# kotaro-kinoshita/yomitoku

Hardware: AMD Instinct MI355X
Metric: pages/sec (DocumentAnalyzer @1600x1200, lite model set) (higher is better)
Workload: dtype f32 held as two scaled fp16 planes per operand on the MFMA pipe: 3 x v_mfma_f32_32x32x16_f16 per product tile (products to 2^-21, below the fp32 accumulation's own rounding), fp32 accumulate, fp32 activations in HBM; attention, LayerNorm, the fused greedy step and every grid-starved launch exact fp3

## Files before the change

yomitoku_amd/csrc/ymk_api.cpp:

```cpp
#include "../../include/ymk.h"
#include "ymk_common.h"
#include "ymk_det.h"
#include "ymk_seq.h"

namespace ymk {
const std::string& last_error();
void dbnet_forward(Model* m, const float* x, int n, int h, int w, float* prob, hipStream_t s);
void parseq_forward(Model* m, const float* x, int B, int W, float* logits, int* out_len, int* ar_steps, hipStream_t s);
void parseq_forward_groups(Model* m, const float* const* x, const int* b, const int* w, int ng, float* logits, int* out_len,
                           int* ar_steps, hipStream_t s);
void parseq_dims(Model* m, int* num_steps, int* num_classes);
Model* create_parseq();
Model* create_rtdetr();
void rtdetr_forward(Model* m, const float* x, int B, int H, int W, float* logits, float* boxes, hipStream_t s);
void row_maxprob(hipStream_t s, const float* logits, int rows, int C, int* ids, float* probs);
void prof_begin();
void prof_end(double* ms, double* flop, int64_t* launches);
double prof_bytes();
int64_t prof_launch_table(double* ms, double* flop, double* bytes, double* products, int64_t capacity);
bool gemm_takes_astat(int M, int K, const ConvW& w, bool with_res, int ld);
bool conv_debug_option(const std::string& key, int value);
bool parseq_debug_option(const std::string& key, int value);
bool decstep_debug_option(const std::string& key, int value);
bool conv_split_debug_option(const std::string& key, int value);
bool conv_split_stat(const std::string& key, long long* value);
void amax_check_counters(long long* out4);
}

struct ymk_model {
  ymk::Model* impl = nullptr;
  int device = 0;
};

#include <dlfcn.h>
namespace {
struct Roctx {
  int (*push)(const char*) = nullptr;
  int (*pop)() = nullptr;
  Roctx() {
    const char* on = std::getenv("YMK_ROCTX");
    if (on == nullptr || on[0] == '\0' || on[0] == '0') return;
    for (const char* name : {"librocprofiler-sdk-roctx.so", "libroctx64.so"}) {
      if (void* h = dlopen(name, RTLD_NOW | RTLD_GLOBAL)) {
        push = reinterpret_cast<int (*)(const char*)>(dlsym(h, "roctxRangePushA"));
        pop = reinterpret_cast<int (*)()>(dlsym(h, "roctxRangePop"));
        if (push && pop) return;
        push = nullptr;
        pop = nullptr;
      }
    }
  }
};
struct RoctxRange {
  explicit RoctxRange(const char* name) {
    static Roctx r;
    pop_ = r.pop;
    if (r.push) (void)r.push(name);
    else pop_ = nullptr;
  }
  ~RoctxRange() {
    if (pop_) (void)pop_();
  }
  int (*pop_)() = nullptr;
};
}

#define YMK_API_BEGIN try {
#define YMK_API_END                                 \
  return 0;                                         \
  }                                                 \
  catch (const std::exception& e) {                 \
    ymk::set_error(e.what());                       \
    return 1;                                       \
  }                                                 \
  catch (...) {                                     \
    ymk::set_error("unknown C++ exception");        \
    return 2;                                       \
  }

extern "C" {

int ymk_version(void) { return 100; }

const char* ymk_last_error(void) { return ymk::last_error().c_str(); }

int ymk_device_count(void) {
  int n = 0;
  if (hipGetDeviceCount(&n) != hipSuccess) return -1;
  return n;
}

ymk_model* ymk_model_create(const char* kind, int device) {
  try {
    YMK_CHECK(kind != nullptr, "kind is null");
    YMK_HIP(hipSetDevice(device));
    std::string k(kind);
    ymk::Model* impl = nullptr;
    if (k == "dbnet") impl = ymk::create_dbnet();
    else if (k == "parseq") impl = ymk::create_parseq();
    else if (k == "rtdetr") impl = ymk::create_rtdetr();
    else throw ymk::Error("unknown model kind: " + k);
    auto* m = new ymk_model();
    m->impl = impl;
    m->device = device;
    return m;
  } catch (const std::exception& e) {
// ... 32 lines not shown
int ymk_model_finalize(ymk_model* m) {
  YMK_API_BEGIN
  RoctxRange roctx_range("ymk_model_finalize");
  YMK_CHECK(m, "null model");
  YMK_HIP(hipSetDevice(m->device));
  m->impl->finalize();
  m->impl->prebuild_split();
  if (!ymk::debug_hazard_no_finalize_sync()) YMK_HIP(hipDeviceSynchronize());
  YMK_API_END
}

int ymk_model_reserve(ymk_model* m, int n, int h, int w, void* stream) {
  YMK_API_BEGIN
  RoctxRange roctx_range("ymk_model_reserve");
  YMK_CHECK(m && m->impl, "null argument");
  YMK_HIP(hipSetDevice(m->device));
  m->impl->reserve(n, h, w, (hipStream_t)stream);
  YMK_API_END
}

int64_t ymk_model_weight_bytes(const ymk_model* m) { return m ? (int64_t)m->impl->pool.bytes() : -1; }
int64_t ymk_model_workspace_bytes(const ymk_model* m) { return m ? (int64_t)m->impl->arena.capacity() : -1; }

int ymk_dbnet_forward(ymk_model* m, const float* x_dev, int n, int h, int w, float* prob_dev, void* stream) {
  YMK_API_BEGIN
  RoctxRange roctx_range("ymk_dbnet_forward");
  YMK_CHECK(m && x_dev && prob_dev, "null argument");
  YMK_HIP(hipSetDevice(m->device));
  ymk::dbnet_forward(m->impl, x_dev, n, h, w, prob_dev, (hipStream_t)stream);
  YMK_API_END
}

int ymk_parseq_dims(ymk_model* m, int* num_steps, int* num_classes) {
  YMK_API_BEGIN
  YMK_CHECK(m && num_steps && num_classes, "null argument");
  ymk::parseq_dims(m->impl, num_steps, num_classes);
  YMK_API_END
}

int ymk_parseq_forward(ymk_model* m, const float* x_dev, int b, int w, float* logits_dev, int* out_len, int* ar_steps,
                       void* stream) {
  YMK_API_BEGIN
  RoctxRange roctx_range("ymk_parseq_forward");
  YMK_CHECK(m && x_dev && logits_dev && out_len && ar_steps, "null argument");
  YMK_HIP(hipSetDevice(m->device));
  ymk::parseq_forward(m->impl, x_dev, b, w, logits_dev, out_len, ar_steps, (hipStream_t)stream);
  YMK_API_END
}

int ymk_parseq_forward_groups(ymk_model* m, const float* const* x_dev, const int* b, const int* w, int n_groups,
                              float* logits_dev, int* out_len, int* ar_steps, void* stream) {
  YMK_API_BEGIN
  RoctxRange roctx_range("ymk_parseq_forward_groups");
  YMK_CHECK(m && x_dev && b && w && logits_dev && out_len && ar_steps, "null argument");
  YMK_HIP(hipSetDevice(m->device));
  ymk::parseq_forward_groups(m->impl, x_dev, b, w, n_groups, logits_dev, out_len, ar_steps, (hipStream_t)stream);
  YMK_API_END
}

int ymk_parseq_token_stats(const float* logits_dev, int rows, int num_classes, int* ids_dev, float* probs_dev,
                           void* stream) {
  YMK_API_BEGIN
  RoctxRange roctx_range("ymk_parseq_token_stats");
  YMK_CHECK(logits_dev && ids_dev && probs_dev, "null argument");
  ymk::row_maxprob((hipStream_t)stream, logits_dev, rows, num_classes, ids_dev, probs_dev);
  YMK_API_END
}

int ymk_rtdetr_forward(ymk_model* m, const float* x_dev, int b, int h, int w, float* logits_dev, float* boxes_dev,
                       void* stream) {
  YMK_API_BEGIN
  RoctxRange roctx_range("ymk_rtdetr_forward");
  YMK_CHECK(m && x_dev && logits_dev && boxes_dev, "null argument");
  YMK_HIP(hipSetDevice(m->device));
  ymk::rtdetr_forward(m->impl, x_dev, b, h, w, logits_dev, boxes_dev, (hipStream_t)stream);
  YMK_API_END
}

int ymk_debug_option(const char* key, int value) {
  YMK_API_BEGIN
  YMK_CHECK(key != nullptr, "null key");
  const std::string k(key);
  YMK_CHECK(ymk::conv_debug_option(k, value) || ymk::parseq_debug_option(k, value) || ymk::decstep_debug_option(k, value) ||
                ymk::conv_split_debug_option(k, value),
            "unknown debug option: " + k);
  YMK_API_END
}

int ymk_stat(const char* key, int64_t* value) {
  YMK_API_BEGIN
  YMK_CHECK(key != nullptr && value != nullptr, "null argument");
  long long v = 0;
  YMK_CHECK(ymk::conv_split_stat(std::string(key), &v) || ymk::runtime_stat(std::string(key), &v), std::string("unknown counter: ") + key);
  *value = v;
  YMK_API_END
}

int ymk_amax_check_counters(int64_t* out4) {
  YMK_API_BEGIN
  YMK_CHECK(out4 != nullptr, "null argument");
  long long v[4];
  ymk::amax_check_counters(v);
  for (int i = 0; i < 4; ++i) out4[i] = v[i];
  YMK_API_END
}

int ymk_prof_begin(void) {
  YMK_API_BEGIN
  ymk::prof_begin();
  YMK_API_END
}

int ymk_prof_end(double* conv_ms, double* conv_flop, int64_t* conv_launches) {
  YMK_API_BEGIN
  YMK_CHECK(conv_ms && conv_flop && conv_launches, "null argument");
  ymk::prof_end(conv_ms, conv_flop, conv_launches);
  YMK_API_END
}

int ymk_prof_bytes(double* conv_bytes) {
  YMK_API_BEGIN
  YMK_CHECK(conv_bytes, "null argument");
  *conv_bytes = ymk::prof_bytes();
  YMK_API_END
}

int ymk_prof_launch_table(double* ms, double* flop, double* bytes, double* mfma_products, int64_t capacity, int64_t* count) {
  YMK_API_BEGIN
  YMK_CHECK(count != nullptr && capacity >= 0 && (capacity == 0 || (ms && flop && bytes && mfma_products)), "null argument");
  *count = ymk::prof_launch_table(ms, flop, bytes, mfma_products, capacity);
  YMK_API_END
}

int ymk_op_conv2d(const float* x_dev, int n, int h, int w, int c, const float* w_host_oihw, int cout, int cin, int kh,
                  int kw, const float* scale_host, const float* bias_host, const float* res_dev, int stride, int pad,
                  int dil, int act, int tap4, float* y_dev, void* stream) {
  YMK_API_BEGIN
  using namespace ymk;
  DevicePool pool;
  ConvW cw;
  cw.cout = cout;
  cw.cin = tap4 ? 4 : cin;
  cw.kh = kh;
  cw.kw = kw;
  cw.mode = tap4 ? 1 : 0;
  std::vector<float> panel;
  pack_conv_weight(w_host_oihw, cout, cin, kh, kw, tap4 != 0, panel, cw.kpad, cw.ctiles);
  cw.w = pool.upload(panel);
  if (scale_host) cw.scale = pool.upload(scale_host, cout);
  if (bias_host) cw.bias = pool.upload(bias_host, cout);
  Tensor in{const_cast<float*>(x_dev), n, h, w, c, c};
  const int oh = conv_out_dim(h, kh, stride, pad, dil), ow = conv_out_dim(w, kw, stride, pad, dil);
  Tensor out{y_dev, n, oh, ow, cout, cout};
  Tensor res{const_cast<float*>(res_dev), n, oh, ow, cout, cout};
  ConvArgs a;
  a.stride = stride;
  a.pad = pad;
  a.dil = dil;
  a.act = act;
  a.res = res_dev ? &res : nullptr;
  SplitCtxOwner split_ctx;
  ConvSplitScope scope(-1, split_ctx.get(), 0);
  conv2d((hipStream_t)stream, in, cw, a, out);
  YMK_HIP(hipStreamSynchronize((hipStream_t)stream));
  YMK_API_END
}

int ymk_op_conv1x1_astat(const float* x_dev, int m, int c, const float* w_host_oc, int cout, const float* scale_host,
                         const float* bias_host, const float* res_dev, int act, const float* ln_g_host, const float* ln_b_host, float ln_eps,
                         float* y_dev, int reps, float* kernel_ms, void* stream) {
  YMK_API_BEGIN
  using namespace ymk;
  YMK_CHECK(x_dev && w_host_oc && y_dev && m > 0 && c > 0 && cout > 0, "bad argument");
  YMK_CHECK((ln_g_host == nullptr) == (ln_b_host == nullptr), "LayerNorm: gamma and beta come together");
  hipStream_t s = (hipStream_t)stream;
  DevicePool pool;
// ... 295 lines not shown
```

yomitoku_amd/csrc/ymk_seq.h:

```cpp
#pragma once
#include "ymk_common.h"

namespace ymk {

void layernorm(hipStream_t s, const float* x, int ldx, int in_rows_mod, const float* g, const float* b, float eps,
               float* y, int ldy, int M, int D);
void add_pos_embed(hipStream_t s, float* x, const float* pos, int B, int gh, int gw, int full_gw, int D);

struct SeqTab {
  const int *qoff = nullptr, *qlen = nullptr, *koff = nullptr, *klen = nullptr;
};

void flash_attention(hipStream_t s, const float* q, const float* k, const float* v, float* o, int B, int H, int Lq, int Lk,
                     int hd, int ldq, int ldk, int ldv, int ldo, long bsq, long bsk, long bsv, long bso, float scale,
                     const SeqTab* tab = nullptr, const unsigned* amax_q = nullptr, const unsigned* amax_k = nullptr,
                     const unsigned* amax_v = nullptr);
void small_attention(hipStream_t s, const float* q, const float* k, const float* v, float* o, int B, int H, int Lq, int Lk,
                     int hd, int ldq, int ldk, int ldv, int ldo, long bsq, long bsk, long bsv, long bso, float scale,
                     const unsigned char* mask_qk, int ld_mask, const unsigned char* kpm, int ld_kpm,
                     const SeqTab* tab = nullptr);
void init_decode(hipStream_t s, int* tok, int ld_tok, int* state, int bos_id, int pad_id, int B);

void ctx_embed_ln(hipStream_t s, const int* tok, int ld_tok, int pos0, int npos, const float* emb, const float* posq,
                  const float* g, const float* be, float eps, float* out, int out_rows, int D, int B);
void greedy_step(hipStream_t s, const float* logits, long ld_b, int C, int step, int num_steps, int* tok, int* raw,
                 int ld_tok, int* state, int eos_id, int rep_on, int period_max, int min_run_p1, int min_repeats,
                 int* not_done, const int* prev_not_done, int* arrived, int* host_flag, int B, const int* gid = nullptr,
                 int* gopen = nullptr, int ng = 1, int partials = 0);
void publish_open(hipStream_t s, const int* not_done, const int* prev_not_done, int* host_flag);
void refine_prep(hipStream_t s, const int* raw, int ld_tok, int S, int bos_id, int eos_id, int* tok2, unsigned char* kpm,
                 int B, const int* gid = nullptr, const int* gsteps = nullptr);
void row_argmax(hipStream_t s, const float* logits, int rows, int C, int* out);
void rep_cut(hipStream_t s, float* logits, long ld_b, int C, int S, const int* state, int eos_id, int B);
void row_maxprob(hipStream_t s, const float* logits, int rows, int C, int* ids, float* probs);
void fill_i32(hipStream_t s, int* p, int v, size_t n);

}
```

yomitoku_amd/csrc/ymk_seq.hip:

```cpp
#include "ymk_common.h"
#include "ymk_seq.h"

namespace ymk {

typedef float f32x16 __attribute__((ext_vector_type(16)));
typedef float f32x4 __attribute__((ext_vector_type(4)));

__device__ __forceinline__ float wave_sum(float v) {
#pragma unroll
  for (int o = 32; o > 0; o >>= 1) v += __shfl_xor(v, o, 64);
  return v;
}
__device__ __forceinline__ float wave_max(float v) {
#pragma unroll
  for (int o = 32; o > 0; o >>= 1) v = fmaxf(v, __shfl_xor(v, o, 64));
  return v;
}

__global__ void k_layernorm(const float* __restrict__ x, int ldx, int in_rows_mod, const float* __restrict__ g,
                            const float* __restrict__ b, float eps, float* __restrict__ y, int ldy, int M, int D) {
  const int row = blockIdx.x * (blockDim.x >> 6) + (threadIdx.x >> 6);
  const int lane = threadIdx.x & 63;
  if (row >= M) return;
  const float* xr = x + (size_t)(in_rows_mod > 0 ? row % in_rows_mod : row) * ldx;
  float4 v[4];
  const int nv = D >> 2;
  float s = 0.f;
#pragma unroll
  for (int i = 0; i < 4; ++i) {
    const int c = lane + 64 * i;
    if (c < nv) {
      v[i] = *reinterpret_cast<const float4*>(xr + c * 4);
      s += (v[i].x + v[i].y) + (v[i].z + v[i].w);
    }
  }
  const float mean = wave_sum(s) / (float)D;
  float q = 0.f;
#pragma unroll
  for (int i = 0; i < 4; ++i) {
    const int c = lane + 64 * i;
    if (c < nv) {
      const float a = v[i].x - mean, bb = v[i].y - mean, cc = v[i].z - mean, d = v[i].w - mean;
      q += (a * a + bb * bb) + (cc * cc + d * d);
    }
  }
  const float rstd = 1.f / sqrtf(wave_sum(q) / (float)D + eps);
#pragma unroll
  for (int i = 0; i < 4; ++i) {
    const int c = lane + 64 * i;
    if (c < nv) {
      const float4 gg = *reinterpret_cast<const float4*>(g + c * 4);
      const float4 be = *reinterpret_cast<const float4*>(b + c * 4);
      float4 o;
      o.x = (v[i].x - mean) * rstd * gg.x + be.x;
      o.y = (v[i].y - mean) * rstd * gg.y + be.y;
      o.z = (v[i].z - mean) * rstd * gg.z + be.z;
      o.w = (v[i].w - mean) * rstd * gg.w + be.w;
      *reinterpret_cast<float4*>(y + (size_t)row * ldy + c * 4) = o;
    }
  }
}
void layernorm(hipStream_t s, const float* x, int ldx, int in_rows_mod, const float* g, const float* b, float eps,
               float* y, int ldy, int M, int D) {
  YMK_CHECK(D % 4 == 0 && D <= 1024, "layernorm: D must be a multiple of 4, <= 1024");
  if (M == 0) return;
  hipLaunchKernelGGL(k_layernorm, dim3((M + 3) / 4), dim3(256), 0, s, x, ldx, in_rows_mod, g, b, eps, y, ldy, M, D);
  YMK_HIP(hipGetLastError());
}

__global__ void k_add_pos(float* __restrict__ x, const float* __restrict__ pos, int gh, int gw, int full_gw, int D4,
                          size_t total) {
  for (size_t i = (size_t)blockIdx.x * blockDim.x + threadIdx.x; i < total; i += (size_t)gridDim.x * blockDim.x) {
    const int c4 = (int)(i % D4);
    const size_t tok = i / D4;
    const int cc = (int)(tok % gw);
    const int rr = (int)((tok / gw) % gh);
    float4 v = reinterpret_cast<float4*>(x)[i];
    const float4 p = reinterpret_cast<const float4*>(pos)[(size_t)(rr * full_gw + cc) * D4 + c4];
    v.x += p.x; v.y += p.y; v.z += p.z; v.w += p.w;
    reinterpret_cast<float4*>(x)[i] = v;
  }
}
void add_pos_embed(hipStream_t s, float* x, const float* pos, int B, int gh, int gw, int full_gw, int D) {
  const size_t total = (size_t)B * gh * gw * (D / 4);
// ... 85 lines not shown
      *reinterpret_cast<f32x4*>(Ks + row * LDH + c4 * 4) = rk[i];
      *reinterpret_cast<f32x4*>(Vs + row * LDH + c4 * 4) = rv[i];
    }
  };

  const int ntiles = (Lk + KT - 1) / KT;
  load_kv(0);
  store_kv(0);
  __syncthreads();
  for (int tt = 0; tt < ntiles; ++tt) {
    const int buf = tt & 1;
    if (tt + 1 < ntiles) load_kv((tt + 1) * KT);
    const float* Ks = lds + buf * (2 * KT * LDH);
    const float* Vs = Ks + KT * LDH;
#pragma unroll
    for (int sub = 0; sub < (q0 < Lq ? KT / 32 : 0); ++sub) {
      const int kbase = tt * KT + sub * 32;
      if (kbase >= Lk) break;
      f32x16 sacc;
#pragma unroll
      for (int r = 0; r < 16; ++r) sacc[r] = 0.f;
      const float* kr = Ks + (sub * 32 + li) * LDH + lh * 4;
#pragma unroll
      for (int kc = 0; kc < NKC; ++kc) {
        const f32x4 kf = *reinterpret_cast<const f32x4*>(kr + kc * 8);
        sacc = __builtin_amdgcn_mfma_f32_32x32x2f32(kf.x, qf[kc].x, sacc, 0, 0, 0);
        sacc = __builtin_amdgcn_mfma_f32_32x32x2f32(kf.y, qf[kc].y, sacc, 0, 0, 0);
        sacc = __builtin_amdgcn_mfma_f32_32x32x2f32(kf.z, qf[kc].z, sacc, 0, 0, 0);
        sacc = __builtin_amdgcn_mfma_f32_32x32x2f32(kf.w, qf[kc].w, sacc, 0, 0, 0);
      }
      float mt = -INFINITY;
#pragma unroll
      for (int r = 0; r < 16; ++r) {
        const int key = kbase + (r & 3) + 8 * (r >> 2) + 4 * lh;
        if (key >= Lk) sacc[r] = -INFINITY;
        mt = fmaxf(mt, sacc[r]);
      }
      mt = fmaxf(mt, __shfl_xor(mt, 32, 64));
      const float m_new = fmaxf(m_run, mt);
      const float alpha = __expf(m_run - m_new);
      float ps = 0.f;
#pragma unroll
      for (int r = 0; r < 16; ++r) {
        sacc[r] = __expf(sacc[r] - m_new);
        ps += sacc[r];
      }
      ps += __shfl_xor(ps, 32, 64);
      l_run = l_run * alpha + ps;
      m_run = m_new;
#pragma unroll
      for (int dc = 0; dc < NDC; ++dc) {
#pragma unroll
        for (int r = 0; r < 16; ++r) oacc[dc][r] *= alpha;
        const float* vr = Vs + (sub * 32 + 4 * lh) * LDH + dc * 32 + li;
#pragma unroll
        for (int r = 0; r < 16; ++r) {
          const float vf = vr[((r & 3) + 8 * (r >> 2)) * LDH];
          oacc[dc] = __builtin_amdgcn_mfma_f32_32x32x2f32(vf, sacc[r], oacc[dc], 0, 0, 0);
        }
      }
    }
    if (tt + 1 < ntiles) store_kv(buf ^ 1);
    __syncthreads();
  }
  const int qi = q0 + li;
  if (qi < Lq) {
    const float inv = 1.f / l_run;
    float* orow = ob + (size_t)qi * p.ldo;
#pragma unroll
    for (int dc = 0; dc < NDC; ++dc)
#pragma unroll
      for (int g = 0; g < 4; ++g) {
        f32x4 w;
        w.x = oacc[dc][4 * g + 0] * inv;
        w.y = oacc[dc][4 * g + 1] * inv;
        w.z = oacc[dc][4 * g + 2] * inv;
        w.w = oacc[dc][4 * g + 3] * inv;
        if (dc * 32 + 8 * g + 4 * lh < HDR) *reinterpret_cast<f32x4*>(orow + dc * 32 + 8 * g + 4 * lh) = w;
      }
  }
}

typedef _Float16 ah16x2 __attribute__((ext_vector_type(2)));
typedef _Float16 ah16x8 __attribute__((ext_vector_type(8)));
typedef float af32x2 __attribute__((ext_vector_type(2)));

__device__ __forceinline__ float2 attn_f16_scales(unsigned amax_bits) {
  int e = (int)(amax_bits >> 23);
  e = e < 27 ? 27 : (e > 227 ? 227 : e);
  float2 r;
  r.x = __uint_as_float((unsigned)(268 - e) << 23);
  r.y = __uint_as_float((unsigned)(e - 14) << 23);
  return r;
}
__device__ __forceinline__ void attn_split8(const float (&x)[8], float sc, ah16x8& hi, ah16x8& lo) {
  ah16x2 h[4], l[4];
#pragma unroll
  for (int i = 0; i < 4; ++i) {
    af32x2 v = {x[2 * i] * sc, x[2 * i + 1] * sc};
    h[i] = __builtin_convertvector(v, ah16x2);
    v -= __builtin_convertvector(h[i], af32x2);
    l[i] = __builtin_convertvector(v, ah16x2);
  }
  hi = ah16x8{h[0].x, h[0].y, h[1].x, h[1].y, h[2].x, h[2].y, h[3].x, h[3].y};
  lo = ah16x8{l[0].x, l[0].y, l[1].x, l[1].y, l[2].x, l[2].y, l[3].x, l[3].y};
}

template <int HD, int HDR = HD>
__global__ __launch_bounds__(256, (HD <= 32 ? 3 : (HD <= 64 ? 2 : 1))) void k_flash_attn_f16(AttnP p) {
  constexpr int KT = 64;
  constexpr int LDH = HD + 4;
  constexpr int NKS = HDR / 16;
  constexpr int NDC = HD / 32;
  constexpr int LPT = (KT * HDR / 4) / 256;
  static_assert(HD % 32 == 0 && HDR % 16 == 0 && HDR <= HD && (KT * HDR / 4) % 256 == 0, "head dim");
  __shared__ __attribute__((aligned(16))) float lds[2 * 2 * KT * LDH];

  const int t = threadIdx.x, wv = t >> 6, lane = t & 63, li = lane & 31, lh = lane >> 5;
  const int b = blockIdx.z, h = blockIdx.y;
  const int q0 = blockIdx.x * 128 + wv * 32;
  const float* qb = p.q + (size_t)b * p.bsq + h * HDR;
  const float* kb = p.k + (size_t)b * p.bsk + h * HDR;
  const float* vb = p.v + (size_t)b * p.bsv + h * HDR;
  float* ob = p.o + (size_t)b * p.bso + h * HDR;
  int Lq = p.Lq, Lk = p.Lk;
  if (p.koff) {
    const size_t r = (size_t)p.koff[b];
    kb = p.k + r * p.ldk + h * HDR;
    vb = p.v + r * p.ldv + h * HDR;
    Lk = p.klen[b];
  }
  if (p.qoff) {
    const size_t r = (size_t)p.qoff[b];
    qb = p.q + r * p.ldq + h * HDR;
    ob = p.o + r * p.ldo + h * HDR;
    Lq = p.qlen[b];
  }
  if ((int)blockIdx.x * 128 >= Lq) return;

  const float2 cq = attn_f16_scales((unsigned)__builtin_amdgcn_readfirstlane((int)amax_read(p.amax_q, t)));
  const float2 ck = attn_f16_scales((unsigned)__builtin_amdgcn_readfirstlane((int)amax_read(p.amax_k, t)));
  const float2 cv = attn_f16_scales((unsigned)__builtin_amdgcn_readfirstlane((int)amax_read(p.amax_v, t)));
  const float s_q = cq.x, s_k = ck.x, s_v = cv.x;
  const float s_unscale = cq.y * ck.y;
  const float o_unscale = cv.y * (1.f / 16384.f);

  ah16x8 qh[NKS], ql[NKS];
  {
    const int qi = min(q0 + li, Lq - 1);
    const float* qr = qb + (size_t)qi * p.ldq;
#pragma unroll
    for (int ks = 0; ks < NKS; ++ks) {
      const f32x4 a = *reinterpret_cast<const f32x4*>(qr + ks * 16 + lh * 8);
      const f32x4 c = *reinterpret_cast<const f32x4*>(qr + ks * 16 + lh * 8 + 4);
      const float x[8] = {a.x * p.scale, a.y * p.scale, a.z * p.scale, a.w * p.scale, c.x * p.scale, c.y * p.scale, c.z * p.scale, c.w * p.scale};
      attn_split8(x, s_q, qh[ks], ql[ks]);
    }
  }

  f32x16 oacc[NDC];
#pragma unroll
  for (int dc = 0; dc < NDC; ++dc)
#pragma unroll
    for (int r = 0; r < 16; ++r) oacc[dc][r] = 0.f;
  float m_run = -INFINITY, l_run = 0.f;

  f32x4 rk[LPT], rv[LPT];
  auto load_kv = [&](int k0) {
#pragma unroll
    for (int i = 0; i < LPT; ++i) {
      const int idx = t + 256 * i;
      const int row = idx / (HDR / 4), c4 = idx - row * (HDR / 4);
      const int key = min(k0 + row, Lk - 1);
      rk[i] = *reinterpret_cast<const f32x4*>(kb + (size_t)key * p.ldk + c4 * 4);
      rv[i] = *reinterpret_cast<const f32x4*>(vb + (size_t)key * p.ldv + c4 * 4);
    }
  };
  auto store_kv = [&](int buf) {
    float* Ks = lds + buf * (2 * KT * LDH);
    float* Vs = Ks + KT * LDH;
#pragma unroll
    for (int i = 0; i < LPT; ++i) {
      const int idx = t + 256 * i;
      const int row = idx / (HDR / 4), c4 = idx - row * (HDR / 4);
      *reinterpret_cast<f32x4*>(Ks + row * LDH + c4 * 4) = rk[i];
      *reinterpret_cast<f32x4*>(Vs + row * LDH + c4 * 4) = rv[i];
    }
  };

  const int ntiles = (Lk + KT - 1) / KT;
  load_kv(0);
  store_kv(0);
  __syncthreads();
  for (int tt = 0; tt < ntiles; ++tt) {
    const int buf = tt & 1;
    if (tt + 1 < ntiles) load_kv((tt + 1) * KT);
    const float* Ks = lds + buf * (2 * KT * LDH);
    const float* Vs = Ks + KT * LDH;
#pragma unroll
    for (int sub = 0; sub < (q0 < Lq ? KT / 32 : 0); ++sub) {
      const int kbase = tt * KT + sub * 32;
      if (kbase >= Lk) break;
      f32x16 sacc;
#pragma unroll
      for (int r = 0; r < 16; ++r) sacc[r] = 0.f;
      const float* kr = Ks + (sub * 32 + li) * LDH + lh * 8;
#pragma unroll
      for (int ks = 0; ks < NKS; ++ks) {
        const f32x4 a = *reinterpret_cast<const f32x4*>(kr + ks * 16);
        const f32x4 c = *reinterpret_cast<const f32x4*>(kr + ks * 16 + 4);
        const float x[8] = {a.x, a.y, a.z, a.w, c.x, c.y, c.z, c.w};
        ah16x8 kh, kl;
        attn_split8(x, s_k, kh, kl);
        sacc = __builtin_amdgcn_mfma_f32_32x32x16_f16(kl, qh[ks], sacc, 0, 0, 0);
        sacc = __builtin_amdgcn_mfma_f32_32x32x16_f16(kh, ql[ks], sacc, 0, 0, 0);
        sacc = __builtin_amdgcn_mfma_f32_32x32x16_f16(kh, qh[ks], sacc, 0, 0, 0);
      }
      float mt = -INFINITY;
#pragma unroll
      for (int r = 0; r < 16; ++r) {
        const int key = kbase + (r & 3) + 8 * (r >> 2) + 4 * lh;
        sacc[r] = key >= Lk ? -INFINITY : sacc[r] * s_unscale;
        mt = fmaxf(mt, sacc[r]);
      }
      mt = fmaxf(mt, __shfl_xor(mt, 32, 64));
      const float m_new = fmaxf(m_run, mt);
      const float alpha = __expf(m_run - m_new);
      float ps = 0.f;
#pragma unroll
      for (int r = 0; r < 16; ++r) {
        sacc[r] = __expf(sacc[r] - m_new);
        ps += sacc[r];
      }
      ps += __shfl_xor(ps, 32, 64);
      l_run = l_run * alpha + ps;
      m_run = m_new;
      ah16x8 ph[2], pl[2];
#pragma unroll
      for (int j = 0; j < 2; ++j) {
        const float x[8] = {sacc[8 * j], sacc[8 * j + 1], sacc[8 * j + 2], sacc[8 * j + 3], sacc[8 * j + 4], sacc[8 * j + 5], sacc[8 * j + 6], sacc[8 * j + 7]};
        attn_split8(x, 16384.f, ph[j], pl[j]);
      }
#pragma unroll
      for (int dc = 0; dc < NDC; ++dc) {
#pragma unroll
        for (int r = 0; r < 16; ++r) oacc[dc][r] *= alpha;
        const float* vr = Vs + (sub * 32 + 4 * lh) * LDH + dc * 32 + li;
#pragma unroll
        for (int j = 0; j < 2; ++j) {
          float x[8];
#pragma unroll
          for (int e = 0; e < 8; ++e) {
            const int r = 8 * j + e;
            x[e] = vr[((r & 3) + 8 * (r >> 2)) * LDH];
          }
          ah16x8 vh, vl;
          attn_split8(x, s_v, vh, vl);
          oacc[dc] = __builtin_amdgcn_mfma_f32_32x32x16_f16(vl, ph[j], oacc[dc], 0, 0, 0);
          oacc[dc] = __builtin_amdgcn_mfma_f32_32x32x16_f16(vh, pl[j], oacc[dc], 0, 0, 0);
          oacc[dc] = __builtin_amdgcn_mfma_f32_32x32x16_f16(vh, ph[j], oacc[dc], 0, 0, 0);
        }
      }
    }
    if (tt + 1 < ntiles) store_kv(buf ^ 1);
    __syncthreads();
  }
  const int qi = q0 + li;
  if (qi < Lq) {
    const float inv = o_unscale / l_run;
    float* orow = ob + (size_t)qi * p.ldo;
#pragma unroll
    for (int dc = 0; dc < NDC; ++dc)
#pragma unroll
      for (int g = 0; g < 4; ++g) {
        f32x4 w;
        w.x = oacc[dc][4 * g + 0] * inv;
        w.y = oacc[dc][4 * g + 1] * inv;
        w.z = oacc[dc][4 * g + 2] * inv;
        w.w = oacc[dc][4 * g + 3] * inv;
        if (dc * 32 + 8 * g + 4 * lh < HDR) *reinterpret_cast<f32x4*>(orow + dc * 32 + 8 * g + 4 * lh) = w;
      }
  }
}

void flash_attention(hipStream_t s, const float* q, const float* k, const float* v, float* o, int B, int H, int Lq, int Lk,
                     int hd, int ldq, int ldk, int ldv, int ldo, long bsq, long bsk, long bsv, long bso, float scale,
                     const SeqTab* tab, const unsigned* amax_q, const unsigned* amax_k, const unsigned* amax_v) {
  if (B == 0 || Lq == 0) return;
  YMK_CHECK(Lk > 0, "attention: no keys");
  YMK_CHECK(ldq % 4 == 0 && ldk % 4 == 0 && ldv % 4 == 0 && ldo % 4 == 0, "attention: strides must be multiples of 4");
  AttnP p{q, k, v, o, ldq, ldk, ldv, ldo, bsq, bsk, bsv, bso, Lq, Lk, H, scale, nullptr, nullptr, nullptr, nullptr, amax_q, amax_k, amax_v};
  if (tab) {
    p.qoff = tab->qoff;
    p.qlen = tab->qlen;
    p.koff = tab->koff;
    p.klen = tab->klen;
    YMK_CHECK((p.qoff == nullptr) == (p.qlen == nullptr) && (p.koff == nullptr) == (p.klen == nullptr), "attention: offset and length tables come in pairs");
  }
  dim3 grid((Lq + 127) / 128, H, B);
  const bool f16 = amax_q && amax_k && amax_v && scale <= 1.f && scale > 0.f && conv_effective_split() == SPLIT_F16X2 && ldq % 4 == 0;
  if (f16 && (hd == 32 || hd == 64 || hd == 96 || hd == 48)) {
    if (hd == 32) hipLaunchKernelGGL(k_flash_attn_f16<32>, grid, dim3(256), 0, s, p);
    else if (hd == 64) hipLaunchKernelGGL(k_flash_attn_f16<64>, grid, dim3(256), 0, s, p);
    else if (hd == 96) hipLaunchKernelGGL(k_flash_attn_f16<96>, grid, dim3(256), 0, s, p);
    else hipLaunchKernelGGL((k_flash_attn_f16<64, 48>), grid, dim3(256), 0, s, p);
    YMK_HIP(hipGetLastError());
    return;
  }
  if (hd == 32) hipLaunchKernelGGL(k_flash_attn<32>, grid, dim3(256), 0, s, p);
  else if (hd == 64) hipLaunchKernelGGL(k_flash_attn<64>, grid, dim3(256), 0, s, p);
  else if (hd == 96) hipLaunchKernelGGL(k_flash_attn<96>, grid, dim3(256), 0, s, p);
  else if (hd == 48) hipLaunchKernelGGL((k_flash_attn<64, 48>), grid, dim3(256), 0, s, p);
  else {
    YMK_CHECK(Lk <= 1024 && hd <= 128, "attention: head dim " + std::to_string(hd) + " is only supported for <= 1024 keys per sample");
    small_attention(s, q, k, v, o, B, H, Lq, Lk, hd, ldq, ldk, ldv, ldo, bsq, bsk, bsv, bso, scale, nullptr, 0, nullptr, 0, tab);
    return;
  }
  YMK_HIP(hipGetLastError());
}

struct SmallAttnP {
  const float *q, *k, *v;
  float* o;
  int ldq, ldk, ldv, ldo;
  long bsq, bsk, bsv, bso;
  int Lq, Lk, H, hd;
  float scale;
  const unsigned char* mask_qk;
  int ld_mask;
  const unsigned char* kpm;
  int ld_kpm;
  const int *koff, *klen;
  const int *qoff, *qlen;
  int vec4;
};
__global__ __launch_bounds__(64) void k_small_attn(SmallAttnP p) {
  __shared__ float prob[1024];
  __shared__ float qs[128];
  const int lane = threadIdx.x;
  const int qi = blockIdx.x, h = blockIdx.y, b = blockIdx.z;
  if (p.qoff && qi >= p.qlen[b]) return;
  const size_t qrow0 = p.qoff ? (size_t)p.qoff[b] : 0;
  const float* qr = (p.qoff ? p.q + qrow0 * p.ldq : p.q + (size_t)b * p.bsq) + (size_t)qi * p.ldq + h * p.hd;
  for (int d = lane; d < p.hd; d += 64) qs[d] = qr[d] * p.scale;
  __syncthreads();
  const float* kb = p.k + (size_t)b * p.bsk + h * p.hd;
  const float* vb = p.v + (size_t)b * p.bsv + h * p.hd;
  int Lk = p.Lk;
  if (p.koff) {
    kb = p.k + (size_t)p.koff[b] * p.ldk + h * p.hd;
    vb = p.v + (size_t)p.koff[b] * p.ldv + h * p.hd;
    Lk = p.klen[b];
  }
  float mx = -INFINITY;
  for (int k = lane; k < Lk; k += 64) {
    bool blocked = false;
    if (p.mask_qk) blocked = p.mask_qk[(size_t)qi * p.ld_mask + k] != 0;
    if (p.kpm) blocked = blocked || p.kpm[(size_t)b * p.ld_kpm + k] != 0;
    float sc = -INFINITY;
    if (!blocked) {
      const float* kr = kb + (size_t)k * p.ldk;
      float a = 0.f;
      if (p.vec4) {
        for (int d = 0; d < p.hd; d += 4) {
          const float4 kk = *reinterpret_cast<const float4*>(kr + d);
          a += qs[d] * kk.x + qs[d + 1] * kk.y + qs[d + 2] * kk.z + qs[d + 3] * kk.w;
        }
      } else {
        for (int d = 0; d < p.hd; ++d) a += qs[d] * kr[d];
      }
      sc = a;
    }
    prob[k] = sc;
    mx = fmaxf(mx, sc);
  }
  mx = wave_max(mx);
  float sum = 0.f;
  for (int k = lane; k < Lk; k += 64) {
    const float e = __expf(prob[k] - mx);
    prob[k] = e;
    sum += e;
  }
  sum = wave_sum(sum);
  __syncthreads();
// ... 370 lines not shown
```

Baseline: 129.0.

## Stage K/V tiles as pre-split fp16 hi/lo planes in LDS for flash attention

Adds a flash-attention kernel variant that splits each K and V tile into scaled fp16 high and low planes once, when it is written to LDS. V is stored transposed in MFMA operand order, and the next tile's global loads are double-buffered into registers while the current tile computes. The goal is to stop every wave from re-splitting fp32 K/V on each read and to overlap global loads with MFMA work. In exchange it uses more LDS per block, which may limit occupancy, and it is on by default behind a debug toggle.

```diff
diff --git a/yomitoku_amd/csrc/ymk_api.cpp b/yomitoku_amd/csrc/ymk_api.cpp
--- a/yomitoku_amd/csrc/ymk_api.cpp
+++ b/yomitoku_amd/csrc/ymk_api.cpp
@@ -22,6 +22,8 @@
 bool conv_debug_option(const std::string& key, int value);
 bool parseq_debug_option(const std::string& key, int value);
 bool decstep_debug_option(const std::string& key, int value);
+bool seq_debug_option(const std::string& key, int value);
+bool seq_stat(const std::string& key, long long* value);
 bool conv_split_debug_option(const std::string& key, int value);
 bool conv_split_stat(const std::string& key, long long* value);
 void amax_check_counters(long long* out4);
@@ -220,7 +222,7 @@
   YMK_CHECK(key != nullptr, "null key");
   const std::string k(key);
   YMK_CHECK(ymk::conv_debug_option(k, value) || ymk::parseq_debug_option(k, value) || ymk::decstep_debug_option(k, value) ||
-                ymk::conv_split_debug_option(k, value),
+                ymk::conv_split_debug_option(k, value) || ymk::seq_debug_option(k, value),
             "unknown debug option: " + k);
   YMK_API_END
 }
@@ -229,7 +231,7 @@
   YMK_API_BEGIN
   YMK_CHECK(key != nullptr && value != nullptr, "null argument");
   long long v = 0;
-  YMK_CHECK(ymk::conv_split_stat(std::string(key), &v) || ymk::runtime_stat(std::string(key), &v), std::string("unknown counter: ") + key);
+  YMK_CHECK(ymk::conv_split_stat(std::string(key), &v) || ymk::runtime_stat(std::string(key), &v) || ymk::seq_stat(std::string(key), &v), std::string("unknown counter: ") + key);
   *value = v;
   YMK_API_END
 }
diff --git a/yomitoku_amd/csrc/ymk_seq.h b/yomitoku_amd/csrc/ymk_seq.h
--- a/yomitoku_amd/csrc/ymk_seq.h
+++ b/yomitoku_amd/csrc/ymk_seq.h
@@ -15,6 +15,8 @@
                      int hd, int ldq, int ldk, int ldv, int ldo, long bsq, long bsk, long bsv, long bso, float scale,
                      const SeqTab* tab = nullptr, const unsigned* amax_q = nullptr, const unsigned* amax_k = nullptr,
                      const unsigned* amax_v = nullptr);
+bool seq_debug_option(const std::string& key, int value);
+bool seq_stat(const std::string& key, long long* value);
 void small_attention(hipStream_t s, const float* q, const float* k, const float* v, float* o, int B, int H, int Lq, int Lk,
                      int hd, int ldq, int ldk, int ldv, int ldo, long bsq, long bsk, long bsv, long bso, float scale,
                      const unsigned char* mask_qk, int ld_mask, const unsigned char* kpm, int ld_kpm,
diff --git a/yomitoku_amd/csrc/ymk_seq.hip b/yomitoku_amd/csrc/ymk_seq.hip
--- a/yomitoku_amd/csrc/ymk_seq.hip
+++ b/yomitoku_amd/csrc/ymk_seq.hip
@@ -1,5 +1,6 @@
 #include "ymk_common.h"
 #include "ymk_seq.h"
+#include <atomic>
 
 namespace ymk {
 
@@ -251,6 +252,7 @@
 }
 
 typedef _Float16 ah16x2 __attribute__((ext_vector_type(2)));
+typedef _Float16 ah16x4 __attribute__((ext_vector_type(4)));
 typedef _Float16 ah16x8 __attribute__((ext_vector_type(8)));
 typedef float af32x2 __attribute__((ext_vector_type(2)));
 
@@ -452,6 +454,251 @@
   }
 }
 
+__device__ __forceinline__ void attn_split2(float a, float b, float sc, ah16x2& h, ah16x2& l) {
+  af32x2 v = {a * sc, b * sc};
+  h = __builtin_convertvector(v, ah16x2);
+  v -= __builtin_convertvector(h, af32x2);
+  l = __builtin_convertvector(v, ah16x2);
+}
+__host__ __device__ constexpr int attn_vt_pos(int kk) { return (kk & ~15) + ((kk >> 2) & 1) * 8 + ((kk >> 3) & 1) * 4 + (kk & 3); }
+
+template <int C4>
+__host__ __device__ constexpr int attn_v_item_kp(int idx) { return ((idx >> 5) / (C4 / 4)) * 8 + ((idx >> 2) & 7); }
+template <int C4>
+__host__ __device__ constexpr int attn_v_item_c4(int idx) { return ((idx >> 5) % (C4 / 4)) * 4 + (idx & 3); }
+
+template <int HD, int HDR = HD>
+__global__ __launch_bounds__(256, (HD <= 32 ? 3 : (HD <= 64 ? 2 : 1))) void k_flash_attn_f16_planes(AttnP p) {
+  constexpr int KT = 64;
+  constexpr int LDK = HDR + 8;
+  constexpr int LDV = KT + 8;
+  constexpr int NKS = HDR / 16;
+  constexpr int NDC = HD / 32;
+  constexpr int C4 = HDR / 4;
+  constexpr int LPT = (KT * C4) / 256;
+  constexpr int NPAIR = (KT / 2) * C4;
+  constexpr int PPT = (NPAIR + 255) / 256;
+  constexpr int BUF = 2 * KT * LDK + 2 * HD * LDV;
+  static_assert(HD % 32 == 0 && HDR % 16 == 0 && HDR <= HD && (KT * C4) % 256 == 0 && C4 % 4 == 0, "head dim");
+  static_assert((LDK / 8) % 2 == 1 && (LDV / 8) % 2 == 1, "row strides: 16 bytes times an odd number");
+  static_assert((HD <= 32 ? 3 : (HD <= 64 ? 2 : 1)) * 2 * BUF * 2 <= 160 * 1024, "LDS: the blocks per CU of __launch_bounds__ must fit");
+  __shared__ __attribute__((aligned(16))) _Float16 lds[2 * BUF];
+
+  const int t = threadIdx.x, wv = t >> 6, lane = t & 63, li = lane & 31, lh = lane >> 5;
+  const int b = blockIdx.z, h = blockIdx.y;
+  const int q0 = blockIdx.x * 128 + wv * 32;
+  const float* qb = p.q + (size_t)b * p.bsq + h * HDR;
+  const float* kb = p.k + (size_t)b * p.bsk + h * HDR;
+  const float* vb = p.v + (size_t)b * p.bsv + h * HDR;
+  float* ob = p.o + (size_t)b * p.bso + h * HDR;
+  int Lq = p.Lq, Lk = p.Lk;
+  if (p.koff) {
+    const size_t r = (size_t)p.koff[b];
+    kb = p.k + r * p.ldk + h * HDR;
+    vb = p.v + r * p.ldv + h * HDR;
+    Lk = p.klen[b];
+  }
+  if (p.qoff) {
+    const size_t r = (size_t)p.qoff[b];
+    qb = p.q + r * p.ldq + h * HDR;
+    ob = p.o + r * p.ldo + h * HDR;
+    Lq = p.qlen[b];
+  }
+  if ((int)blockIdx.x * 128 >= Lq) return;
+
+  const float2 cq = attn_f16_scales((unsigned)__builtin_amdgcn_readfirstlane((int)amax_read(p.amax_q, t)));
+  const float2 ck = attn_f16_scales((unsigned)__builtin_amdgcn_readfirstlane((int)amax_read(p.amax_k, t)));
+  const float2 cv = attn_f16_scales((unsigned)__builtin_amdgcn_readfirstlane((int)amax_read(p.amax_v, t)));
+  const float s_q = cq.x, s_k = ck.x, s_v = cv.x;
+  const float s_unscale = cq.y * ck.y;
+  const float o_unscale = cv.y * (1.f / 16384.f);
+
+  ah16x8 qh[NKS], ql[NKS];
+  {
+    const int qi = min(q0 + li, Lq - 1);
+    const float* qr = qb + (size_t)qi * p.ldq;
+#pragma unroll
+    for (int ks = 0; ks < NKS; ++ks) {
+      const f32x4 a = *reinterpret_cast<const f32x4*>(qr + ks * 16 + lh * 8);
+      const f32x4 c = *reinterpret_cast<const f32x4*>(qr + ks * 16 + lh * 8 + 4);
+      const float x[8] = {a.x * p.scale, a.y * p.scale, a.z * p.scale, a.w * p.scale, c.x * p.scale, c.y * p.scale, c.z * p.scale, c.w * p.scale};
+      attn_split8(x, s_q, qh[ks], ql[ks]);
+    }
+  }
+
+  f32x16 oacc[NDC];
+#pragma unroll
+  for (int dc = 0; dc < NDC; ++dc)
+#pragma unroll
+    for (int r = 0; r < 16; ++r) oacc[dc][r] = 0.f;
+  float m_run = -INFINITY, l_run = 0.f;
+
+  f32x4 rk[LPT], rv[PPT][2];
+  auto load_kv = [&](int k0) {
+#pragma unroll
+    for (int i = 0; i < LPT; ++i) {
+      const int idx = t + 256 * i;
+      const int row = idx / C4, c4 = idx - row * C4;
+      const int key = min(k0 + row, Lk - 1);
+      rk[i] = *reinterpret_cast<const f32x4*>(kb + (size_t)key * p.ldk + c4 * 4);
+    }
+#pragma unroll
+    for (int i = 0; i < PPT; ++i) {
+      const int idx = t + 256 * i;
+      if (NPAIR % 256 == 0 || idx < NPAIR) {
+        const int kp = attn_v_item_kp<C4>(idx), c4 = attn_v_item_c4<C4>(idx);
+#pragma unroll
+        for (int u = 0; u < 2; ++u) {
+          const int key = min(k0 + 2 * kp + u, Lk - 1);
+          rv[i][u] = *reinterpret_cast<const f32x4*>(vb + (size_t)key * p.ldv + c4 * 4);
+        }
+      }
+    }
+  };
+  auto store_kv = [&](int buf) {
+    _Float16* Kh = lds + buf * BUF;
+    _Float16* Kl = Kh + KT * LDK;
+    _Float16* Vh = Kl + KT * LDK;
+    _Float16* Vl = Vh + HD * LDV;
+#pragma unroll
+    for (int i = 0; i < LPT; ++i) {
+      const int idx = t + 256 * i;
+      const int row = idx / C4, c4 = idx - row * C4;
+      ah16x2 h0, l0, h1, l1;
+      attn_split2(rk[i].x, rk[i].y, s_k, h0, l0);
+      attn_split2(rk[i].z, rk[i].w, s_k, h1, l1);
+      *reinterpret_cast<ah16x4*>(Kh + row * LDK + c4 * 4) = ah16x4{h0.x, h0.y, h1.x, h1.y};
+      *reinterpret_cast<ah16x4*>(Kl + row * LDK + c4 * 4) = ah16x4{l0.x, l0.y, l1.x, l1.y};
+    }
+#pragma unroll
+    for (int i = 0; i < PPT; ++i) {
+      const int idx = t + 256 * i;
+      if (NPAIR % 256 == 0 || idx < NPAIR) {
+        const int kp = attn_v_item_kp<C4>(idx), c4 = attn_v_item_c4<C4>(idx);
+        const int col = attn_vt_pos(2 * kp);
+#pragma unroll
+        for (int dd = 0; dd < 4; ++dd) {
+          ah16x2 hh, ll;
+          attn_split2(rv[i][0][dd], rv[i][1][dd], s_v, hh, ll);
+          *reinterpret_cast<ah16x2*>(Vh + (c4 * 4 + dd) * LDV + col) = hh;
+          *reinterpret_cast<ah16x2*>(Vl + (c4 * 4 + dd) * LDV + col) = ll;
+        }
+      }
+    }
+  };
+
+  const int ntiles = (Lk + KT - 1) / KT;
+  load_kv(0);
+  store_kv(0);
+  __syncthreads();
+  for (int tt = 0; tt < ntiles; ++tt) {
+    const int buf = tt & 1;
+    if (tt + 1 < ntiles) load_kv((tt + 1) * KT);
+    const _Float16* Kh = lds + buf * BUF;
+    const _Float16* Kl = Kh + KT * LDK;
+    const _Float16* Vh = Kl + KT * LDK;
+    const _Float16* Vl = Vh + HD * LDV;
+#pragma unroll
+    for (int sub = 0; sub < (q0 < Lq ? KT / 32 : 0); ++sub) {
+      const int kbase = tt * KT + sub * 32;
+      if (kbase >= Lk) break;
+      f32x16 sacc;
+#pragma unroll
+      for (int r = 0; r < 16; ++r) sacc[r] = 0.f;
+      const int ko = (sub * 32 + li) * LDK + lh * 8;
+#pragma unroll
+      for (int ks = 0; ks < NKS; ++ks) {
+        const ah16x8 kh = *reinterpret_cast<const ah16x8*>(Kh + ko + ks * 16);
+        const ah16x8 kl = *reinterpret_cast<const ah16x8*>(Kl + ko + ks * 16);
+        sacc = __builtin_amdgcn_mfma_f32_32x32x16_f16(kl, qh[ks], sacc, 0, 0, 0);
+        sacc = __builtin_amdgcn_mfma_f32_32x32x16_f16(kh, ql[ks], sacc, 0, 0, 0);
+        sacc = __builtin_amdgcn_mfma_f32_32x32x16_f16(kh, qh[ks], sacc, 0, 0, 0);
+      }
+      float mt = -INFINITY;
+      if (kbase + 32 > Lk) {
+#pragma unroll
+        for (int r = 0; r < 16; ++r) {
+          const int key = kbase + (r & 3) + 8 * (r >> 2) + 4 * lh;
+          sacc[r] = key >= Lk ? -INFINITY : sacc[r] * s_unscale;
+          mt = fmaxf(mt, sacc[r]);
+        }
+      } else {
+#pragma unroll
+        for (int r = 0; r < 16; ++r) {
+          sacc[r] = sacc[r] * s_unscale;
+          mt = fmaxf(mt, sacc[r]);
+        }
+      }
+      mt = fmaxf(mt, __shfl_xor(mt, 32, 64));
+      const float m_new = fmaxf(m_run, mt);
+      const float alpha = __expf(m_run - m_new);
+      float ps = 0.f;
+#pragma unroll
+      for (int r = 0; r < 16; ++r) {
+        sacc[r] = __expf(sacc[r] - m_new);
+        ps += sacc[r];
+      }
+      ps += __shfl_xor(ps, 32, 64);
+      l_run = l_run * alpha + ps;
+      m_run = m_new;
+      ah16x8 ph[2], pl[2];
+#pragma unroll
+      for (int j = 0; j < 2; ++j) {
+        const float x[8] = {sacc[8 * j], sacc[8 * j + 1], sacc[8 * j + 2], sacc[8 * j + 3], sacc[8 * j + 4], sacc[8 * j + 5], sacc[8 * j + 6], sacc[8 * j + 7]};
+        attn_split8(x, 16384.f, ph[j], pl[j]);
+      }
+      const bool rescale = __ballot(alpha != 1.f) != 0ull;
+#pragma unroll
+      for (int dc = 0; dc < NDC; ++dc) {
+        if (rescale) {
+#pragma unroll
+          for (int r = 0; r < 16; ++r) oacc[dc][r] *= alpha;
+        }
+        const int vo = (dc * 32 + li) * LDV + sub * 32 + lh * 8;
+#pragma unroll
+        for (int j = 0; j < 2; ++j) {
+          const ah16x8 vh = *reinterpret_cast<const ah16x8*>(Vh + vo + j * 16);
+          const ah16x8 vl = *reinterpret_cast<const ah16x8*>(Vl + vo + j * 16);
+          oacc[dc] = __builtin_amdgcn_mfma_f32_32x32x16_f16(vl, ph[j], oacc[dc], 0, 0, 0);
+          oacc[dc] = __builtin_amdgcn_mfma_f32_32x32x16_f16(vh, pl[j], oacc[dc], 0, 0, 0);
+          oacc[dc] = __builtin_amdgcn_mfma_f32_32x32x16_f16(vh, ph[j], oacc[dc], 0, 0, 0);
+        }
+      }
+    }
+    if (tt + 1 < ntiles) store_kv(buf ^ 1);
+    __syncthreads();
+  }
+  const int qi = q0 + li;
+  if (qi < Lq) {
+    const float inv = o_unscale / l_run;
+    float* orow = ob + (size_t)qi * p.ldo;
+#pragma unroll
+    for (int dc = 0; dc < NDC; ++dc)
+#pragma unroll
+      for (int g = 0; g < 4; ++g) {
+        f32x4 w;
+        w.x = oacc[dc][4 * g + 0] * inv;
+        w.y = oacc[dc][4 * g + 1] * inv;
+        w.z = oacc[dc][4 * g + 2] * inv;
+        w.w = oacc[dc][4 * g + 3] * inv;
+        if (dc * 32 + 8 * g + 4 * lh < HDR) *reinterpret_cast<f32x4*>(orow + dc * 32 + 8 * g + 4 * lh) = w;
+      }
+  }
+}
+
+static std::atomic<int> g_attn_kv_planes{1};
+static std::atomic<long long> g_attn_kv_planes_launches{0};
+bool seq_debug_option(const std::string& key, int value) {
+  if (key == "attn_kv_planes") g_attn_kv_planes = value;
+  else return false;
+  return true;
+}
+bool seq_stat(const std::string& key, long long* value) {
+  if (key == "attn_kv_planes_launches") *value = g_attn_kv_planes_launches.load(std::memory_order_relaxed);
+  else return false;
+  return true;
+}
+
 void flash_attention(hipStream_t s, const float* q, const float* k, const float* v, float* o, int B, int H, int Lq, int Lk,
                      int hd, int ldq, int ldk, int ldv, int ldo, long bsq, long bsk, long bsv, long bso, float scale,
                      const SeqTab* tab, const unsigned* amax_q, const unsigned* amax_k, const unsigned* amax_v) {
@@ -468,6 +715,15 @@
   }
   dim3 grid((Lq + 127) / 128, H, B);
   const bool f16 = amax_q && amax_k && amax_v && scale <= 1.f && scale > 0.f && conv_effective_split() == SPLIT_F16X2 && ldq % 4 == 0;
+  if (f16 && (hd == 32 || hd == 64 || hd == 96 || hd == 48) && g_attn_kv_planes.load(std::memory_order_relaxed) != 0) {
+    if (hd == 32) hipLaunchKernelGGL(k_flash_attn_f16_planes<32>, grid, dim3(256), 0, s, p);
+    else if (hd == 64) hipLaunchKernelGGL(k_flash_attn_f16_planes<64>, grid, dim3(256), 0, s, p);
+    else if (hd == 96) hipLaunchKernelGGL(k_flash_attn_f16_planes<96>, grid, dim3(256), 0, s, p);
+    else hipLaunchKernelGGL((k_flash_attn_f16_planes<64, 48>), grid, dim3(256), 0, s, p);
+    YMK_HIP(hipGetLastError());
+    g_attn_kv_planes_launches.fetch_add(1, std::memory_order_relaxed);
+    return;
+  }
   if (f16 && (hd == 32 || hd == 64 || hd == 96 || hd == 48)) {
     if (hd == 32) hipLaunchKernelGGL(k_flash_attn_f16<32>, grid, dim3(256), 0, s, p);
     else if (hd == 64) hipLaunchKernelGGL(k_flash_attn_f16<64>, grid, dim3(256), 0, s, p);
```

Result: no change. 131.1, median of 6 (+1.6%).

## Pre-split K/V into fp16 hi/lo planes in LDS once per tile

Applied to the files above, without the earlier changes.

K and V tiles are now split into scaled fp16 hi/lo halves when they are stored to shared memory, rather than being re-split by every wave from fp32 LDS on each read. V is stored transposed in an MFMA-friendly permuted order, so each wave loads its operands as packed 8-wide fp16 vectors. The change also adds a fast path that skips key masking on full tiles, skips the oacc rescale when no lane's running max changed, and raises the HD=32 occupancy hint. The LDS footprint per buffer changes, and the V gather pattern during the global load is more complex.

```diff
diff --git a/yomitoku_amd/csrc/ymk_seq.hip b/yomitoku_amd/csrc/ymk_seq.hip
--- a/yomitoku_amd/csrc/ymk_seq.hip
+++ b/yomitoku_amd/csrc/ymk_seq.hip
@@ -251,6 +251,7 @@
 }
 
 typedef _Float16 ah16x2 __attribute__((ext_vector_type(2)));
+typedef _Float16 ah16x4 __attribute__((ext_vector_type(4)));
 typedef _Float16 ah16x8 __attribute__((ext_vector_type(8)));
 typedef float af32x2 __attribute__((ext_vector_type(2)));
 
@@ -262,32 +263,43 @@
   r.y = __uint_as_float((unsigned)(e - 14) << 23);
   return r;
 }
+__device__ __forceinline__ void attn_split2(af32x2 v, ah16x2& h, ah16x2& l) {
+  h = __builtin_convertvector(v, ah16x2);
+  v -= __builtin_convertvector(h, af32x2);
+  l = __builtin_convertvector(v, ah16x2);
+}
 __device__ __forceinline__ void attn_split8(const float (&x)[8], float sc, ah16x8& hi, ah16x8& lo) {
   ah16x2 h[4], l[4];
 #pragma unroll
-  for (int i = 0; i < 4; ++i) {
-    af32x2 v = {x[2 * i] * sc, x[2 * i + 1] * sc};
-    h[i] = __builtin_convertvector(v, ah16x2);
-    v -= __builtin_convertvector(h[i], af32x2);
-    l[i] = __builtin_convertvector(v, ah16x2);
-  }
+  for (int i = 0; i < 4; ++i) attn_split2(af32x2{x[2 * i] * sc, x[2 * i + 1] * sc}, h[i], l[i]);
   hi = ah16x8{h[0].x, h[0].y, h[1].x, h[1].y, h[2].x, h[2].y, h[3].x, h[3].y};
   lo = ah16x8{l[0].x, l[0].y, l[1].x, l[1].y, l[2].x, l[2].y, l[3].x, l[3].y};
 }
 
+__device__ __forceinline__ int attn_vpos(int kk) {
+  const int w = kk & 15;
+  return (kk & ~15) + ((w >> 2) & 1) * 8 + (w & 3) + 4 * (w >> 3);
+}
+constexpr int kAttnF16QWaves = 4;
+
 template <int HD, int HDR = HD>
-__global__ __launch_bounds__(256, (HD <= 32 ? 3 : (HD <= 64 ? 2 : 1))) void k_flash_attn_f16(AttnP p) {
+__global__ __launch_bounds__(256, (HD <= 32 ? 4 : (HD <= 64 ? 2 : 1))) void k_flash_attn_f16(AttnP p) {
   constexpr int KT = 64;
-  constexpr int LDH = HD + 4;
+  constexpr int LDKH = 2 * HD + 8;
+  constexpr int LDVH = 2 * KT + 8;
+  constexpr int BUFH = KT * LDKH + HD * LDVH;
   constexpr int NKS = HDR / 16;
   constexpr int NDC = HD / 32;
   constexpr int LPT = (KT * HDR / 4) / 256;
+  constexpr int NVI = (KT / 2) * (HDR / 4);
+  constexpr int VPT = (NVI + 255) / 256;
+  constexpr int QW = kAttnF16QWaves;
   static_assert(HD % 32 == 0 && HDR % 16 == 0 && HDR <= HD && (KT * HDR / 4) % 256 == 0, "head dim");
-  __shared__ __attribute__((aligned(16))) float lds[2 * 2 * KT * LDH];
+  __shared__ __attribute__((aligned(16))) _Float16 lds[2 * BUFH];
 
   const int t = threadIdx.x, wv = t >> 6, lane = t & 63, li = lane & 31, lh = lane >> 5;
   const int b = blockIdx.z, h = blockIdx.y;
-  const int q0 = blockIdx.x * 128 + wv * 32;
+  const int q0 = blockIdx.x * (32 * QW) + wv * 32;
   const float* qb = p.q + (size_t)b * p.bsq + h * HDR;
   const float* kb = p.k + (size_t)b * p.bsk + h * HDR;
   const float* vb = p.v + (size_t)b * p.bsv + h * HDR;
@@ -305,7 +317,8 @@
     ob = p.o + r * p.ldo + h * HDR;
     Lq = p.qlen[b];
   }
-  if ((int)blockIdx.x * 128 >= Lq) return;
+  if ((int)blockIdx.x * (32 * QW) >= Lq) return;
+  const bool live = wv < QW && q0 < Lq;
 
   const float2 cq = attn_f16_scales((unsigned)__builtin_amdgcn_readfirstlane((int)amax_read(p.amax_q, t)));
   const float2 ck = attn_f16_scales((unsigned)__builtin_amdgcn_readfirstlane((int)amax_read(p.amax_k, t)));
@@ -315,7 +328,7 @@
   const float o_unscale = cv.y * (1.f / 16384.f);
 
   ah16x8 qh[NKS], ql[NKS];
-  {
+  if (live) {
     const int qi = min(q0 + li, Lq - 1);
     const float* qr = qb + (size_t)qi * p.ldq;
 #pragma unroll
@@ -334,7 +347,7 @@
     for (int r = 0; r < 16; ++r) oacc[dc][r] = 0.f;
   float m_run = -INFINITY, l_run = 0.f;
 
-  f32x4 rk[LPT], rv[LPT];
+  f32x4 rk[LPT], rv[2 * VPT];
   auto load_kv = [&](int k0) {
 #pragma unroll
     for (int i = 0; i < LPT; ++i) {
@@ -342,18 +355,46 @@
       const int row = idx / (HDR / 4), c4 = idx - row * (HDR / 4);
       const int key = min(k0 + row, Lk - 1);
       rk[i] = *reinterpret_cast<const f32x4*>(kb + (size_t)key * p.ldk + c4 * 4);
-      rv[i] = *reinterpret_cast<const f32x4*>(vb + (size_t)key * p.ldv + c4 * 4);
+    }
+#pragma unroll
+    for (int i = 0; i < VPT; ++i) {
+      const int idx = t + 256 * i;
+      if (NVI % 256 == 0 || idx < NVI) {
+        const int kp = ((idx >> 5) & 3) * 8 + (idx & 7), c4 = (idx >> 7) * 4 + ((idx >> 3) & 3);
+        const int key0 = min(k0 + 2 * kp, Lk - 1), key1 = min(k0 + 2 * kp + 1, Lk - 1);
+        rv[2 * i] = *reinterpret_cast<const f32x4*>(vb + (size_t)key0 * p.ldv + c4 * 4);
+        rv[2 * i + 1] = *reinterpret_cast<const f32x4*>(vb + (size_t)key1 * p.ldv + c4 * 4);
+      }
     }
   };
   auto store_kv = [&](int buf) {
-    float* Ks = lds + buf * (2 * KT * LDH);
-    float* Vs = Ks + KT * LDH;
+    _Float16* Kp = lds + buf * BUFH;
+    _Float16* Vp = Kp + KT * LDKH;
 #pragma unroll
     for (int i = 0; i < LPT; ++i) {
       const int idx = t + 256 * i;
       const int row = idx / (HDR / 4), c4 = idx - row * (HDR / 4);
-      *reinterpret_cast<f32x4*>(Ks + row * LDH + c4 * 4) = rk[i];
-      *reinterpret_cast<f32x4*>(Vs + row * LDH + c4 * 4) = rv[i];
+      ah16x2 h0, l0, h1, l1;
+      attn_split2(af32x2{rk[i].x * s_k, rk[i].y * s_k}, h0, l0);
+      attn_split2(af32x2{rk[i].z * s_k, rk[i].w * s_k}, h1, l1);
+      _Float16* kw = Kp + row * LDKH + c4 * 4;
+      *reinterpret_cast<ah16x4*>(kw) = ah16x4{h0.x, h0.y, h1.x, h1.y};
+      *reinterpret_cast<ah16x4*>(kw + HD) = ah16x4{l0.x, l0.y, l1.x, l1.y};
+    }
+#pragma unroll
+    for (int i = 0; i < VPT; ++i) {
+      const int idx = t + 256 * i;
+      if (NVI % 256 == 0 || idx < NVI) {
+        const int kp = ((idx >> 5) & 3) * 8 + (idx & 7), c4 = (idx >> 7) * 4 + ((idx >> 3) & 3);
+        _Float16* vw = Vp + (c4 * 4) * LDVH + attn_vpos(2 * kp);
+#pragma unroll
+        for (int c = 0; c < 4; ++c) {
+          ah16x2 hh, ll;
+          attn_split2(af32x2{rv[2 * i][c] * s_v, rv[2 * i + 1][c] * s_v}, hh, ll);
+          *reinterpret_cast<ah16x2*>(vw + c * LDVH) = hh;
+          *reinterpret_cast<ah16x2*>(vw + c * LDVH + KT) = ll;
+        }
+      }
     }
   };
 
@@ -364,33 +405,38 @@
   for (int tt = 0; tt < ntiles; ++tt) {
     const int buf = tt & 1;
     if (tt + 1 < ntiles) load_kv((tt + 1) * KT);
-    const float* Ks = lds + buf * (2 * KT * LDH);
-    const float* Vs = Ks + KT * LDH;
-#pragma unroll
-    for (int sub = 0; sub < (q0 < Lq ? KT / 32 : 0); ++sub) {
+    const _Float16* Kp = lds + buf * BUFH;
+    const _Float16* Vp = Kp + KT * LDKH;
+#pragma unroll
+    for (int sub = 0; sub < (live ? KT / 32 : 0); ++sub) {
       const int kbase = tt * KT + sub * 32;
       if (kbase >= Lk) break;
       f32x16 sacc;
 #pragma unroll
       for (int r = 0; r < 16; ++r) sacc[r] = 0.f;
-      const float* kr = Ks + (sub * 32 + li) * LDH + lh * 8;
+      const _Float16* kr = Kp + (sub * 32 + li) * LDKH + lh * 8;
 #pragma unroll
       for (int ks = 0; ks < NKS; ++ks) {
-        const f32x4 a = *reinterpret_cast<const f32x4*>(kr + ks * 16);
-        const f32x4 c = *reinterpret_cast<const f32x4*>(kr + ks * 16 + 4);
-        const float x[8] = {a.x, a.y, a.z, a.w, c.x, c.y, c.z, c.w};
-        ah16x8 kh, kl;
-        attn_split8(x, s_k, kh, kl);
+        const ah16x8 kh = *reinterpret_cast<const ah16x8*>(kr + ks * 16);
+        const ah16x8 kl = *reinterpret_cast<const ah16x8*>(kr + ks * 16 + HD);
         sacc = __builtin_amdgcn_mfma_f32_32x32x16_f16(kl, qh[ks], sacc, 0, 0, 0);
         sacc = __builtin_amdgcn_mfma_f32_32x32x16_f16(kh, ql[ks], sacc, 0, 0, 0);
         sacc = __builtin_amdgcn_mfma_f32_32x32x16_f16(kh, qh[ks], sacc, 0, 0, 0);
       }
       float mt = -INFINITY;
-#pragma unroll
-      for (int r = 0; r < 16; ++r) {
-        const int key = kbase + (r & 3) + 8 * (r >> 2) + 4 * lh;
-        sacc[r] = key >= Lk ? -INFINITY : sacc[r] * s_unscale;
-        mt = fmaxf(mt, sacc[r]);
+      if (kbase + 32 <= Lk) {
+#pragma unroll
+        for (int r = 0; r < 16; ++r) {
+          sacc[r] *= s_unscale;
+          mt = fmaxf(mt, sacc[r]);
+        }
+      } else {
+#pragma unroll
+        for (int r = 0; r < 16; ++r) {
+          const int key = kbase + (r & 3) + 8 * (r >> 2) + 4 * lh;
+          sacc[r] = key >= Lk ? -INFINITY : sacc[r] * s_unscale;
+          mt = fmaxf(mt, sacc[r]);
+        }
       }
       mt = fmaxf(mt, __shfl_xor(mt, 32, 64));
       const float m_new = fmaxf(m_run, mt);
@@ -410,21 +456,18 @@
         const float x[8] = {sacc[8 * j], sacc[8 * j + 1], sacc[8 * j + 2], sacc[8 * j + 3], sacc[8 * j + 4], sacc[8 * j + 5], sacc[8 * j + 6], sacc[8 * j + 7]};
         attn_split8(x, 16384.f, ph[j], pl[j]);
       }
+      const bool rescale = __any(alpha != 1.f);
 #pragma unroll
       for (int dc = 0; dc < NDC; ++dc) {
-#pragma unroll
-        for (int r = 0; r < 16; ++r) oacc[dc][r] *= alpha;
-        const float* vr = Vs + (sub * 32 + 4 * lh) * LDH + dc * 32 + li;
+        if (rescale) {
+#pragma unroll
+          for (int r = 0; r < 16; ++r) oacc[dc][r] *= alpha;
+        }
+        const _Float16* vr = Vp + (dc * 32 + li) * LDVH + sub * 32 + lh * 8;
 #pragma unroll
         for (int j = 0; j < 2; ++j) {
-          float x[8];
-#pragma unroll
-          for (int e = 0; e < 8; ++e) {
-            const int r = 8 * j + e;
-            x[e] = vr[((r & 3) + 8 * (r >> 2)) * LDH];
-          }
-          ah16x8 vh, vl;
-          attn_split8(x, s_v, vh, vl);
+          const ah16x8 vh = *reinterpret_cast<const ah16x8*>(vr + j * 16);
+          const ah16x8 vl = *reinterpret_cast<const ah16x8*>(vr + j * 16 + KT);
           oacc[dc] = __builtin_amdgcn_mfma_f32_32x32x16_f16(vl, ph[j], oacc[dc], 0, 0, 0);
           oacc[dc] = __builtin_amdgcn_mfma_f32_32x32x16_f16(vh, pl[j], oacc[dc], 0, 0, 0);
           oacc[dc] = __builtin_amdgcn_mfma_f32_32x32x16_f16(vh, ph[j], oacc[dc], 0, 0, 0);
@@ -435,7 +478,7 @@
     __syncthreads();
   }
   const int qi = q0 + li;
-  if (qi < Lq) {
+  if (live && qi < Lq) {
     const float inv = o_unscale / l_run;
     float* orow = ob + (size_t)qi * p.ldo;
 #pragma unroll
@@ -469,6 +512,7 @@
   dim3 grid((Lq + 127) / 128, H, B);
   const bool f16 = amax_q && amax_k && amax_v && scale <= 1.f && scale > 0.f && conv_effective_split() == SPLIT_F16X2 && ldq % 4 == 0;
   if (f16 && (hd == 32 || hd == 64 || hd == 96 || hd == 48)) {
+    grid.x = (Lq + 32 * kAttnF16QWaves - 1) / (32 * kAttnF16QWaves);
     if (hd == 32) hipLaunchKernelGGL(k_flash_attn_f16<32>, grid, dim3(256), 0, s, p);
     else if (hd == 64) hipLaunchKernelGGL(k_flash_attn_f16<64>, grid, dim3(256), 0, s, p);
     else if (hd == 96) hipLaunchKernelGGL(k_flash_attn_f16<96>, grid, dim3(256), 0, s, p);
```

Measured after the change: 131.3 before, 132.5 after (median of 2 runs). Within noise of the previous version (+0.9%).
